# JinPLu/VeloxSeg

Hardware: AMD Instinct MI355X
Metric: training patches/s on 128^3 2-mod volumes (fwd+loss+bwd+allreduce+AdamW) (higher is better)
Workload: dtype f32

## Files before the change

include/veloxseg_hip.h:

```cpp
#ifndef VELOXSEG_HIP_H
#define VELOXSEG_HIP_H

#ifdef __cplusplus
extern "C" {
#endif

#define VX_ABI_VERSION 1

int vx_abi_version(void);
const char* vx_last_error(void);

int vx_conv3d_fwd(const float* x, const float* x2, int C1, const float* w, const float* bias, float* y,
                  int B, int Cin, int Di, int Hi, int Wi, int Cout, int K, int S, int P, int G, int ps, void* stream);
int vx_conv3d_bwd_data(const float* dy, const float* w, const float* bias_like, float* dx, float* dx2, int C1,
                       int B, int Cin, int Di, int Hi, int Wi, int Cout, int K, int S, int P, int G, int ps,
                       int accumulate, void* stream);
int vx_conv3d_bwd_weight(const float* x, const float* x2, int C1, const float* dy, float* dw, float* db,
                         int B, int Cin, int Di, int Hi, int Wi, int Cout, int K, int S, int P, int G, int ps, void* stream);

int vx_conv3d_bwd_weight_tiled(const float* x, const float* x2, int C1, const float* dy, float* dw, float* db,
                               int B, int Cin, int Di, int Hi, int Wi, int Cout, int K, int S, int P, int G, int ps, void* stream);
int vx_down_wgrad_ws_floats(int B, int Cin, int Di, int Hi, int Wi, int Cout);
int vx_down_wgrad_mfma(const float* x, const float* dy, float* dw, float* db, float* ws, long ws_floats,
                       int B, int Cin, int Di, int Hi, int Wi, int Cout, void* stream);
// ... 80 lines not shown
int vx_jlc_gk_h(const void* d_o, const void* y1, const void* y3, const void* y5, const float* stats_y, const float* part_t, void* g1, void* g3,
                void* g5, long BC, long V, int h16, void* stream);
int vx_mlp_fwd_h(const void* x, int norm, const double* part, int nparts, float* stats, const float* gamma, const float* beta,
                 const float* w1, const float* b1, const float* w2, const float* b2, float* out, int B, int C, int R, long V, float eps,
                 const void* seed_ptr, unsigned long long site1, float p1, unsigned long long site2, float p2, int h16, void* stream);
int vx_mlp_bwd_h(const void* x, int norm, const float* stats, const float* gamma, const float* beta, const float* w1, const float* b1,
                 const float* w2, const float* dout, void* dx, float* part_out, float* dgamma, float* dbeta, float* dw1, float* db1,
                 float* dw2, float* db2, int B, int C, int R, long V, float eps, const void* seed_ptr, unsigned long long site1, float p1,
                 unsigned long long site2, float p2, int h16, void* stream);

int vx_jlc_tz_ok(int C, int G, int D, int H, int W);
int vx_jlc_tz_ntiles(int C, int G, int D, int H, int W);
int vx_jlc_tz_img_floats(int C, int G);
int vx_jlc_tz_set_pieces(int ns);
int vx_jlc_tz_set_min_voxels(long v);
int vx_jlc_tz_pieces(void);
int vx_jlc_tz_set_debug(int mask);
int vx_jlc_tz_prep(const float* w1, const float* w3, const float* w5, float* img, int C, int G, void* stream);
int vx_jlc_tz_fwd(const float* x, const float* img, const float* b1, const float* b3, const float* b5, float* y1, float* y3, float* y5, double* part,
                  int B, int C, int G, int D, int H, int W, void* stream);
int vx_jlc_tz_bwd(const float* g1, const float* g3, const float* g5, const float* img, const float* w1, const float* d_o, float* dx,
                  int B, int C, int G, int D, int H, int W, void* stream);
int vx_jlc_cl_ok(int C, int G, int D, int H, int W);
int vx_jlc_cl_ntiles(int C, int G, int D, int H, int W);
int vx_jlc_cl_img_floats(int C, int G);
int vx_jlc_cl_set_enabled(int on);
int vx_jlc_cl_prep(const float* w1, const float* w3, const float* w5, float* img, int C, int G, void* stream);
int vx_jlc_cl_fwd(const float* x, const float* img, const float* b1, const float* b3, const float* b5, float* y1, float* y3, float* y5, double* part,
                  int B, int C, int G, int D, int H, int W, void* stream);
int vx_jlc_cl_bwd(const float* g1, const float* g3, const float* g5, const float* img, const float* d_o, float* dx, int B, int C, int G, int D, int H, int W,
                  void* stream);
int vx_jlc_wgrad_tz_ok(int C, int G, int D, int H, int W);
int vx_jlc_wgrad_tz_set_min_voxels(long v);
int vx_jlc_wgrad_tz_set_blocks(int n);
int vx_jlc_wgrad_tz_set_spec(int on);
int vx_jlc_wgrad_tz_set_f16(int on);
int vx_jlc_wgrad_tz(const float* x, const float* g1, const float* g3, const float* g5, float* dw1, float* dw3, float* dw5, int B, int C, int G, int D, int H, int W,
                    void* stream);
int vx_jlc_tz_img_floats_ns(int C, int G, int pieces);
int vx_jlc_tz_prep_ns(const float* w1, const float* w3, const float* w5, float* img, int C, int G, int pieces, void* stream);
int vx_jlc_tz_fwd_ns(const float* x, const float* img, const float* b1, const float* b3, const float* b5, float* y1, float* y3, float* y5, double* part,
                     int B, int C, int G, int D, int H, int W, int pieces, void* stream);
int vx_jlc_tz_bwd_ns(const float* g1, const float* g3, const float* g5, const float* img, const float* w1, const float* d_o, float* dx,
                     int B, int C, int G, int D, int H, int W, int pieces, void* stream);
int vx_jlc_wgrad_tz_ns(const float* x, const float* g1, const float* g3, const float* g5, float* dw1, float* dw3, float* dw5, int B, int C, int G, int D, int H, int W,
                       int pieces, void* stream);
int vx_jlc_tz_fwd_h(const float* x, const float* img, const float* b1, const float* b3, const float* b5, void* y1, void* y3, void* y5, double* part,
                    int B, int C, int G, int D, int H, int W, int pieces, int h16, void* stream);
int vx_jlc_tz_bwd_h(const void* g1, const void* g3, const void* g5, const float* img, const float* w1, const void* d_o, float* dx,
                    int B, int C, int G, int D, int H, int W, int pieces, int h16, void* stream);
int vx_jlc_wgrad_tz_h(const float* x, const void* g1, const void* g3, const void* g5, float* dw1, float* dw3, float* dw5, int B, int C, int G, int D, int H, int W,
                      int pieces, int h16, void* stream);

int vx_in_stats(const float* x, float* stats, double* part_ws, long BC, long V, float eps, void* stream);
int vx_in_apply_fwd(const float* y0, const float* y1, const float* y2, const float* s0, const float* s1, const float* s2,
                    int nk, int act, const float* res, float* out, long BC, long V, void* stream);
int vx_in_bwd(const float* dout, const float* y, const float* stats, int act, float* m_ws, double* part_ws, float* dy, long BC, long V, void* stream);
int vx_in_row_max(void);
int vx_in_row_fwd(const float* y0, const float* y1, const float* y2, float* s0, float* s1, float* s2, int nk, int act, const float* res,
                  float* out, long BC, long V, float eps, void* stream);
int vx_in_row_bwd(const float* dout, const float* y0, const float* y1, const float* y2, const float* s0, const float* s1, const float* s2,
                  int nk, int act, float* d0, float* d1, float* d2, long BC, long V, void* stream);
int vx_in_bwd_db(const float* dout, const float* y, const float* stats, int act, float* m_ws, double* part_ws, float* dy, long BC, long V, float* db, int C, void* stream);
int vx_in_fwd_split(const float* y0, const float* y1, const float* y2, float* s0, float* s1, float* s2, double* part_ws,
                    int nk, int act, const float* res, float* out, long BC, long V, float eps, void* stream);
int vx_in_bwd_split(const float* dout, const float* y0, const float* y1, const float* y2, const float* s0, const float* s1, const float* s2,
                    double* part_ws, int nk, int act, float* dy0, float* dy1, float* dy2, const float* add0, long BC, long V, void* stream);
int vx_in_row_bwd_add(const float* dout, const float* y0, const float* stats0, int act, const float* add0, float* d0, long BC, long V, void* stream);
int vx_in_row_bwd_db(const float* dout, const float* y0, const float* y1, const float* y2, const float* s0, const float* s1, const float* s2,
                     int nk, int act, float* d0, float* d1, float* d2, float* db0, float* db1, float* db2, int C, long BC, long V, void* stream);

int vx_ln_cf_fwd(const float* x, const float* gamma, const float* beta, float* out, int B, int C, long V, float eps, void* stream);
int vx_ln_cf_bwd(const float* x, const float* gamma, const float* dout, float* dx, float* dgamma, float* dbeta, float* ws,
                 int B, int C, long V, float eps, void* stream);
int vx_ln_cf_bwd_add(const float* x, const float* gamma, const float* dout, const float* add, float* dx, float* dgamma, float* dbeta, float* ws,
                     int B, int C, long V, float eps, void* stream);
int vx_ln_cf_bwd_data(const float* x, const float* gamma, const float* dout, const float* add, float* dx, float* ws, int B, int C, long V, float eps, void* stream);
int vx_ln_cf_bwd_param(const float* x, const float* dout, const float* ws, float* dgamma, float* dbeta, int B, int C, long V, void* stream);

int vx_gelu_drop_fwd(const float* a, float* h, long n, const void* seed_ptr, unsigned long long dstream, float p, void* stream);
int vx_gelu_drop_bwd(const float* dh, const float* a, float* da, long n, const void* seed_ptr, unsigned long long dstream, float p, void* stream);
int vx_axpy_drop_fwd(const float* x, const float* z, float* out, float alpha, long n, const void* seed_ptr, unsigned long long dstream, float p, void* stream);
int vx_axpy_drop_bwd(const float* dout, float* dx, float* dz, float alpha, long n, const void* seed_ptr, unsigned long long dstream, float p, void* stream);
int vx_add(const float* a, const float* b, const float* c, float* out, long n, void* stream);
int vx_add_many(const float* const* a, const float* const* b, const float* const* c, float* const* out, const long* n, int count, void* stream);
int vx_channel_sum(const float* dy, float* db, int B, int C, long V, void* stream);
int vx_space_to_depth2(const float* x, float* out, int B, int C, int Dc, int Hc, int Wc, int inverse, void* stream);
int vx_patchify(const float* x, float* out, int B, int C, int d, int h, int w, int K, void* stream);
int vx_patchify_bs(const float* x, long batch_stride, float* out, int B, int C, int d, int h, int w, int K, void* stream);
int vx_patchify_bs_h(const float* x, long batch_stride, void* out, int B, int C, int d, int h, int w, int K, int out_h16, void* stream);
int vx_patch_embed_ok(int Cin, int Cout, int Do, int Ho, int Wo, int K);
int vx_patch_embed_fwd(const float* x, long batch_stride, const float* w, const float* bias, float* y, int B, int Cin, int Cout, int Do, int Ho, int Wo, void* stream);
int vx_patch_embed_bwd_weight(const float* x, long batch_stride, const float* dy, float* dw, float* db, int B, int Cin, int Cout, int Do, int Ho, int Wo, void* stream);

typedef struct VxPwaPlan {
    int grid[3];
    int n[3];
    int heads, nb;
    int small[4][3];
    int nwin[4][3];
    int woff[4];
    int Ntot;
    int l;
} VxPwaPlan;

int vx_pwa_gather_fwd(const float* src, float* tok, const VxPwaPlan* plan, int c, int m, int M, int B, void* stream);
int vx_pwa_gather_bwd(const float* src, const float* dtok, float* dsrc, const VxPwaPlan* plan, int c, int m, int M, int B, void* stream);
int vx_pwa_gather_all_fwd(const float* const* srcs, float* tq, float* tk, float* tv, int* iq, int* ik, int* iv,
                          const VxPwaPlan* plan, int cq, int cv, int M, int B, void* stream);
int vx_pwa_gather_all_bwd(const float* dtq, const float* dtk, const float* dtv, const int* iq, const int* ik, const int* iv, float* const* dsrcs,
                          const VxPwaPlan* plan, int cq, int cv, int M, int B, void* stream);
int vx_pwa_scatter_fwd(const float* tok, float* out, const VxPwaPlan* plan, int c, int m, int M, int B, void* stream);
int vx_pwa_scatter_bwd(const float* dout, float* dtok, const VxPwaPlan* plan, int c, int m, int M, int B, void* stream);
int vx_pwa_scatter_fwd_all(const float* tok, float* const* outs, const VxPwaPlan* plan, int c, int M, int B, void* stream);
int vx_pwa_scatter_bwd_all(const float* const* douts, float* dtok, const VxPwaPlan* plan, int c, int M, int B, void* stream);
int vx_pwa_scatter_bwd_all_w(const float* const* douts, float* dtok, const VxPwaPlan* plan, int c, int M, int B, void* stream);
int vx_pwa_scatter_bwd_all_wz(const float* const* douts, float* dtok, const VxPwaPlan* plan, int c, int M, int B, float* extra_zero, long extra_floats, void* stream);
int vx_pwa_attn_set_fused_bwd(int on);
int vx_pwa_scatter_set_ident(int on);
int vx_pwa_attn_fwd(const float* Q, const float* K, const float* V, const float* table, float* O, float* LSE,
                    const VxPwaPlan* plan, int B, int M, int cq, int cv,
                    const void* seed_ptr, unsigned long long dstream, float p_drop, void* stream);
int vx_pwa_attn_bwd_ws_floats(const VxPwaPlan* plan, int B, int M);
int vx_pwa_attn_bwd_rep_offset(const VxPwaPlan* plan, int B, int M);
int vx_pwa_attn_bwd_mark_rep_zeroed(const float* delta_ws);
int vx_pwa_gather_set_vec(int on);
int vx_pwa_attn_bwd(const float* Q, const float* K, const float* V, const float* table, const float* O, const float* LSE,
                    const float* dO, float* dQ, float* dK, float* dV, float* dtable, float* delta_ws,
                    const VxPwaPlan* plan, int B, int M, int cq, int cv,
                    const void* seed_ptr, unsigned long long dstream, float p_drop, void* stream);
int vx_pwa_attn_bwd_nofold(const float* Q, const float* K, const float* V, const float* table, const float* O, const float* LSE,
                           const float* dO, float* dQ, float* dK, float* dV, float* delta_ws,
                           const VxPwaPlan* plan, int B, int M, int cq, int cv,
                           const void* seed_ptr, unsigned long long dstream, float p_drop, void* stream);
int vx_pwa_attn_bwd_fold(const float* delta_ws, float* dtable, const VxPwaPlan* plan, int B, int M, void* stream);
int vx_pwa_attn_bwd_fold_many(const float* const* delta_ws, float* const* dtables, const VxPwaPlan* const* plans, int count, int B, int M, void* stream);
int vx_pwa_attn_set_split(int S);
int vx_pwa_attn_bwd1_ok(const VxPwaPlan* plan, int B, int M, int cq, int cv);
int vx_pwa_attn_mbits_words(const VxPwaPlan* plan, int B, int M);
int vx_pwa_attn_mbits_useful(const VxPwaPlan* plan, int B, int M, int cq, int cv);
int vx_pwa_attn_set_valu_bits(int on);
int vx_pwa_attn_fwd_mb(const float* q, const float* k, const float* v, const float* table, float* out, float* lse, const VxPwaPlan* plan, int B, int M, int cq, int cv,
                       const void* seed_ptr, unsigned long long dstream, float p_drop, void* mbits, void* stream);
int vx_pwa_attn_bwd_mb(const float* q, const float* k, const float* v, const float* table, const float* out, const float* lse, const float* dout,
                       float* dq, float* dk, float* dv, float* dtable, float* delta_ws, const VxPwaPlan* plan, int B, int M, int cq, int cv,
                       const void* seed_ptr, unsigned long long dstream, float p_drop, const void* mbits, void* stream);
int vx_pwa_attn_bwd_nofold_mb(const float* q, const float* k, const float* v, const float* table, const float* out, const float* lse, const float* dout,
                              float* dq, float* dk, float* dv, float* delta_ws, const VxPwaPlan* plan, int B, int M, int cq, int cv,
                              const void* seed_ptr, unsigned long long dstream, float p_drop, const void* mbits, void* stream);
int vx_pwa_attn_mfma_ok(const VxPwaPlan* plan, int B, int M, int cq, int cv);
int vx_pwa_attn_set_mfma(int on);
int vx_pwa_attn_bwd1h_ok(const VxPwaPlan* plan, int B, int M, int cq, int cv);
int vx_pwa_attn_set_f16_bwd(int on);
int vx_pwa_attn_set_f16_bwd_ragged(int on);
int vx_pwa_attn_set_f16_bwd_m1(int on);
int vx_pwa_attn_set_short(int on);

int vx_seg_loss_fwd(const float* l0, const float* l1, const float* l2, const float* l3, int nh, const void* labels, int lab_kind,
                    double* acc, int B, int C, long V, void* stream);
int vx_sqdiff_sum(const float* a, const float* b, long n, double* acc, void* stream);
int vx_sqdiff_sum_bs(const float* a, const float* b, long n_per_sample, long b_batch_stride, int B, double* acc, void* stream);
int vx_mse_bwd_bs(const float* a, const float* b, long n_per_sample, long b_batch_stride, int B, const float* coef, const float* gout, float* da, void* stream);
int vx_sqdiff_sum_grad_bs(const float* a, const float* b, long n_per_sample, long b_batch_stride, int B, double* acc, float scale, float* da, void* stream);
int vx_sqdiff_sum_grad_bs_h(const void* a, const float* b, long n_per_sample, long b_batch_stride, int B, double* acc, float scale, void* da, int a_h16, void* stream);
int vx_loss_finalize(const double* seg_acc, int nh, int B, int C, long V, const float* head_weights,
                     const double* rc_acc, long n_rc, float w_rc,
                     const float* gram_seg, const float* g0, const float* g1, const float* g2, const float* g3, int M, int Cg, float w_f,
                     float* loss_out, float* coef, void* stream);
int vx_seg_loss_bwd(const float* logits, const void* labels, int lab_kind, const float* coef_head, const float* gout,
                    float* dlogits, int B, int C, long V, void* stream);
int vx_seg_loss_bwd4(const float* lg0, const float* lg1, const float* lg2, const float* lg3, int nh, const void* labels, int lab_kind, const float* coef,
                     int coef_stride, const float* gout, float* dl0, float* dl1, float* dl2, float* dl3, int B, int C, long V, void* stream);
int vx_seg_loss_ds_ok(int C, int D, int H, int W);
int vx_seg_loss_ds_set_columns(int on);
int vx_seg_loss_ds_ws_floats(const int* low_dims, int nh, int B, int C, int D);
int vx_seg_loss_ds_fwd(const float* l0, const float* l1, const float* l2, const float* l3, const int* low_dims, int nh, const void* labels, int lab_kind,
                       double* acc, int B, int C, int D, int H, int W, void* stream);
int vx_seg_loss_ds_bwd(const float* l0, const float* l1, const float* l2, const float* l3, const int* low_dims, int nh, const void* labels, int lab_kind,
                       const float* coef, int coef_stride, const float* gout, float* dl0, float* dl1, float* dl2, float* dl3, float* ws,
                       int B, int C, int D, int H, int W, void* stream);
int vx_seg_loss_ds_h16_ok(const int* low_dims, int nh, int B, int C, int D, int H, int W);
int vx_seg_loss_ds_fwd_h(const void* l0, const float* l1, const float* l2, const float* l3, const int* low_dims, int nh, const void* labels, int lab_kind,
                         double* acc, int B, int C, int D, int H, int W, int l0_h16, void* stream);
int vx_seg_loss_ds_bwd_h(const void* l0, const float* l1, const float* l2, const float* l3, const int* low_dims, int nh, const void* labels, int lab_kind,
                         const float* coef, int coef_stride, const float* gout, void* dl0, float* dl1, float* dl2, float* dl3, float* ws,
                         int B, int C, int D, int H, int W, int l0_h16, void* stream);
int vx_mse_bwd(const float* a, const float* b, const float* coef, const float* gout, float* da, long n, void* stream);
int vx_gram_mse_bwd(const float* gs, const float* g0, const float* g1, const float* g2, const float* g3, int M, const float* coef,
                    const float* gout, float* dgs, float* d0, float* d1, float* d2, float* d3, long n, void* stream);
int vx_gram_fwd(const float* x, float* G, int B, int C, long V, void* stream);
int vx_gram_bwd(const float* x, const float* dG, float* dx, int B, int C, long V, void* stream);
int vx_upsample_trilinear_fwd(const float* x, float* out, long BC, int d, int h, int w, int D, int H, int W, void* stream);
int vx_upsample_trilinear_bwd(const float* dout, float* dx, float* ws, long BC, int d, int h, int w, int D, int H, int W, void* stream);

int vx_upconv_set_mfma4(int on);
int vx_upconv_k2s2_fwd(const float* x, const float* w, const float* bias, float* y, int B, int Ci, int Co, int d, int h, int wd, void* stream);
int vx_upconv_k2s2_bwd_data(const float* dy, const float* w, float* dx, int B, int Ci, int Co, int d, int h, int wd, void* stream);
int vx_upconv_k2s2_wgrad_ok(int Ci, int Co);
int vx_upconv_k2s2_wgrad(const float* x, const float* dy, float* dw, int B, int Ci, int Co, int d, int h, int wd, void* stream);

int vx_adamw_step(float* p, const float* g, float* m, float* v, long n, float lr, float beta1, float beta2, float eps,
                  float weight_decay, long step, float grad_scale, void* stream);

int vx_sw_extract(const float* vol, float* win, int C, int D, int H, int W, int rd, int rh, int rw, int z0, int y0, int x0, void* stream);
int vx_sw_accumulate(const float* win, float* acc, int C, int D, int H, int W, int rd, int rh, int rw, int z0, int y0, int x0, float weight, void* stream);
int vx_sw_finalize(const float* acc, float* out, unsigned char* labels, const float* cz, const float* cy, const float* cx,
                   int C, int D, int H, int W, void* stream);
int vx_argmax_channels(const float* logits, unsigned char* labels, int B, int C, long V, void* stream);
int vx_confusion(const void* pred, int pred_bytes, const void* gt, int gt_bytes, unsigned long long* conf, int B, long V, int NC, void* stream);

int vx_min_value(const float* x, long n, float* out_init_inf, void* stream);
int vx_bbox_gt(const float* x, float thr, int C, int D, int H, int W, int* out6, void* stream);
int vx_label_chunk_count(const void* labels, int lab_bytes, long n, int chunk, int fg, int* counts, void* stream);
int vx_label_kth_in_chunk(const void* labels, int lab_bytes, long n, long chunk_start, int chunk, int fg, int k, long* out_index, void* stream);
int vx_rotate_z(const float* x, float* out, int C, int D, int H, int W, float cos_a, float sin_a, int mode, void* stream);

int vx_conv_mfma_ok(int Cin, int Cout, int D, int H, int W, int K, int S, int P, int G, int ps);
int vx_conv_mfma_set_stem_f16(int on);
int vx_conv_mfma_set_stem_pieces(int np);
int vx_conv_mfma_stem_pieces(void);
int vx_conv_mfma_ws_floats(int Cin, int Cout, int K, int backward);
int vx_conv_mfma_fwd(const float* x, const float* w, const float* bias, float* y, float* ws, int B, int Cin, int D, int H, int W, int Cout, int K, int S, int P,
                     void* stream);
int vx_conv_mfma_fwd_writes_absmax(int Cin, int Cout, int D, int H, int W, int K, int S, int P);
int vx_conv_mfma_fwd_mx(const float* x, const float* w, const float* bias, float* y, float* ws, unsigned* x_absmax, int B, int Cin, int D, int H, int W, int Cout,
                        int K, int S, int P, void* stream);
int vx_conv_mfma_bwd_data(const float* dy, const float* w, float* dx, float* ws, int B, int Cin, int D, int H, int W, int Cout, int K, int S, int P, int accumulate,
                          void* stream);

int vx_expand_split_ws_floats(int Cc, int ns);
int vx_expand_fwd_mfma_split(const float* x, const float* w, const float* bias, float* wt_ws, float* y, int B, int Cc, int D, int H, int W, int ns, void* stream);
int vx_expand_bwd_data_mfma_split(const float* dy_fine, const float* w, float* wt_ws, float* dx, int B, int Cc, int D, int H, int W, int accumulate, int ns, void* stream);
int vx_expand_split_ew_offset(int Cc);
int vx_expand_prep_split22(const float* w, float* wt_fwd, float* wt_bwd, int Cc, void* stream);
int vx_expand_fwd_mfma_split_prepared(const float* x, const float* bias, const float* wt_fwd, float* y, int B, int Cc, int D, int H, int W, void* stream);
int vx_expand_bwd_data_mfma_split_prepared(const float* dy_fine, const float* wt_bwd, const float* ew_fwd, float* dx, int B, int Cc, int D, int H, int W, int accumulate, void* stream);
int vx_expand_bwd_data_mfma_split_ew(const float* dy_fine, const float* w, float* wt_ws, float* dx, int B, int Cc, int D, int H, int W, int accumulate, int ns,
                                     const float* ew_fwd, void* stream);

int vx_ln_pw_ok(int C, int NS, const int* J, long V, int s2d);
int vx_ln_pw_tiles(int B, long V);
int vx_ln_pw_fwd(const void* const* ptrs, int M, int NS, const int* J, int B, int C, long V, float eps, int s2d, int gd, int gh, int gw, void* stream);
int vx_ln_pw_bwd(const void* const* ptrs, int M, int NS, const int* J, int B, int C, long V, float eps, int s2d, int gd, int gh, int gw, void* stream);
int vx_pwa_post_ok(int C, int Cv, int R, long V);
int vx_pwa_post_tiles(int B, long V);
int vx_pwa_post_fwd(const void* const* ptrs, int M, int B, int C, int Cv, int R, long V, float eps, float alpha, const void* seed_ptr, float p_mix, float p_ffn, void* stream);
int vx_pwa_post_bwd(const void* const* ptrs, int M, int B, int C, int Cv, int R, long V, float eps, float alpha, const void* seed_ptr, float p_mix, float p_ffn, void* stream);

int vx_inmlp_ok(int C, int R, long V);
int vx_inmlp_tiles(long V);
int vx_inmlp_fwd(const float* o, const double* part, int nparts, float* stats, const float* w1, const float* b1, const float* w2, const float* b2, float* out,
                 int B, int C, int R, long V, float eps, const void* seed_ptr, unsigned long long site, float p_drop, void* stream);
int vx_inmlp_bwd(const float* o, const float* stats, const float* w1, const float* b1, const float* w2, const float* dout, float* dn, float* part_dn,
                 float* sc_n, float* sc_h, float* sc_da, float* sc_dz, int B, int C, int R, long V, const void* seed_ptr, unsigned long long site, float p_drop,
                 void* stream);
int vx_pw_wgrad_group(const void* const* ptrs, const long* dims, int nj, const void* const* fptrs, const int* fdims, int nf, void* stream);

typedef struct VxTape VxTape;
int vx_tape_build(void* hip_graph, int max_lanes, VxTape** out);
int vx_tape_build_pgo(void* graph, int max_lanes, const float* dur_us, int n, VxTape** out);
int vx_tape_info(const VxTape* tape, int* n_nodes, int* n_kernels, int* n_lanes, int* n_events);
int vx_tape_set_lane_rotation(VxTape* tape, int k);
int vx_tape_replay(VxTape* tape, void* stream);
int vx_tape_free(VxTape* tape);
int vx_tape_flag_set(void* flag, int value, void* stream);
int vx_tape_flag_wait(const void* flag, int value, void* stream);
int vx_tape_set_flags(int on);
int vx_tape_set_flag_timeout_ms(int ms);
int vx_tape_flag_timeouts(void);
int vx_tape_hop(int slot, void* src, void* dst);
int vx_tape_mark(int id, void* stream);
int vx_tape_wait_marker(VxTape* tape, int id, void* stream);
int vx_tape_has_marker(const VxTape* tape, int id);
int vx_tape_profile(VxTape* tape, void* stream, int reps, float* us);
int vx_tape_describe(const VxTape* tape, int* lane, int* grid, int* waits4, char* names, int name_stride);
int vx_tape_waits(const VxTape* tape, int* waits, int stride);
int vx_tape_launch_node(VxTape* tape, int node, void* stream);
int vx_tape_set_fuzz(int seed, float max_us, float prob);
int vx_tape_node_param(const VxTape* tape, int node, int k, int nparams, int size, void* out, int cap, int* got);
int vx_tape_node_kind(const VxTape* tape, int node);
int vx_tape_replay_prefix(VxTape* tape, void* stream, int k);
int vx_tape_lane_stream(void* any_stream, int lane, void** out);
int vx_spin_us(float us, void* stream);
int vx_tape_lanes_distinct(void);
int vx_tape_spin_us(void);
int vx_tape_lane_on_caller_queue(void);
int vx_tape_permute_lanes(const int* perm4);

#ifdef __cplusplus
}
#endif
#endif
```

veloxseg_amd/csrc/pwa_mfma.hip:

```cpp
#include "vx_common.h"
#include <stdlib.h>
#include "../../include/veloxseg_hip.h"

typedef float vx_f32x4 __attribute__((ext_vector_type(4)));
#define VX_MFMA(a, b, c) __builtin_amdgcn_mfma_f32_16x16x4f32((a), (b), (c), 0, 0, 0)
#define VX_DTABLE_REPLICAS 16

struct VxAttnM {
    int BH, heads, Nt, ML, l, M;
    int n[3];
    float scale;
    int lin_cst, Tsz;
    int xcd;
};

__device__ __forceinline__ void vx_am_tables(const VxAttnM& A, const float* __restrict__ table, int a, int* lin, float* bias, int nthr) {
    for (int t = threadIdx.x; t < A.l; t += nthr) {
        const int t2 = t % A.n[2], t1 = (t / A.n[2]) % A.n[1], t0 = t / (A.n[2] * A.n[1]);
        lin[t] = (t0 * (2 * A.n[1] - 1) + t1) * (2 * A.n[2] - 1) + t2;
    }
    for (int k0 = threadIdx.x; k0 < A.Tsz; k0 += nthr * 8) {
        float v[8];
#pragma unroll
        for (int u = 0; u < 8; ++u) { const int k = k0 + u * nthr; v[u] = table[(long)(k < A.Tsz ? k : 0) * A.heads + a]; }
// ... 930 lines not shown
#pragma unroll
            for (int g = 0; g < MF; ++g)
#pragma unroll
                for (int f = 0; f < MF; ++f) mkc[g][f] = mk[g][f];
            if (j + 1 < NTq) load_bits(j + 1);
            float dssum[4] = {0.f, 0.f, 0.f, 0.f};
            bool pv[4];
#pragma unroll
            for (int i = 0; i < 4; ++i) pv[i] = !RAG || (kval && 16 * qt + 4 * qg + i < A.l);
            uint32_t pmh[2][4], pml[2][4], dsh[2][4], dsl[2][4];
            if constexpr (MF == 1) {
#pragma unroll
                for (int e = 2; e < 4; ++e) { pmh[0][e] = 0u; pml[0][e] = 0u; dsh[0][e] = 0u; dsl[0][e] = 0u; }
            }
#pragma unroll
            for (int g = 0; g < MF; ++g) {
                const _Float16* rrow = rq + (g * nq + 16 * j + m) * VX_BH_RS;
                const vx_au4 aS = *reinterpret_cast<const vx_au4*>(rrow + poffS), aP = *reinterpret_cast<const vx_au4*>(rrow + poffP);
                const float4 l4 = *reinterpret_cast<const float4*>(&lse_s[g * nq + 16 * j + 4 * qg]);
                const float4 d4 = *reinterpret_cast<const float4*>(&del_s[g * nq + 16 * j + 4 * qg]);
                const float bl[4] = {bs[0] - l4.x, bs[1] - l4.y, bs[2] - l4.z, bs[3] - l4.w}, del[4] = {d4.x, d4.y, d4.z, d4.w};
                vx_f32x4 sv_[2], dp[2];
#pragma unroll
                for (int f = 0; f < MF; ++f) {
                    sv_[f] = VX_MFMA_H(aS, kop[f], ((vx_f32x4){0.f, 0.f, 0.f, 0.f}));
                    dp[f] = VX_MFMA_H(aP, vop[f], ((vx_f32x4){0.f, 0.f, 0.f, 0.f}));
                }
#pragma unroll
                for (int f = 0; f < MF; ++f) {
                    float pm[4], ds[4];
#pragma unroll
                    for (int i = 0; i < 4; ++i) {
                        float p = __builtin_amdgcn_exp2f(fmaf(sv_[f][i], cS, bl[i]));
                        if (RAG) p = pv[i] ? p : 0.0f;
                        float mkf = 1.0f;
                        if constexpr (DROP) {
                            const uint32_t w = (i < 2) ? mkc[g][f].x : mkc[g][f].y;
                            mkf = ((w >> (m + 16 * (i & 1))) & 1u) ? keepf : 0.0f;
                        }
                        pm[i] = p * mkf;
                        ds[i] = p * fmaf(dp[f][i], mkf, -del[i]);
                        dssum[i] += ds[i];
                    }
                    vx_a_split2(pm[0], pm[1], pmh[f][2 * g], pml[f][2 * g]);
                    vx_a_split2(pm[2], pm[3], pmh[f][2 * g + 1], pml[f][2 * g + 1]);
                    vx_a_split2(ds[0], ds[1], dsh[f][2 * g], dsl[f][2 * g]);
                    vx_a_split2(ds[2], ds[3], dsh[f][2 * g + 1], dsl[f][2 * g + 1]);
                }
                __builtin_amdgcn_wave_barrier();
#pragma unroll
                for (int f = 0; f < MF; ++f)
#pragma unroll
                    for (int i = 0; i < 4; ++i) {
                        const uint32_t h = dsh[f][2 * g + (i >> 1)], l = dsl[f][2 * g + (i >> 1)];
                        tr[f * (16 * TS) + (4 * qg + i) * TS + m] = (i & 1) ? __builtin_amdgcn_perm(l, h, 0x07060302u) : __builtin_amdgcn_perm(l, h, 0x05040100u);
                    }
                __builtin_amdgcn_wave_barrier();
                const vx_au4 r0 = *reinterpret_cast<const vx_au4*>(&tr[m * TS + 4 * qg]);
                const vx_au4 r1 = MF == 2 ? *reinterpret_cast<const vx_au4*>(&tr[16 * TS + m * TS + 4 * qg]) : (vx_au4){0u, 0u, 0u, 0u};
                __builtin_amdgcn_wave_barrier();
                const vx_au4 bh = {__builtin_amdgcn_perm(r0[1], r0[0], 0x05040100u), __builtin_amdgcn_perm(r0[3], r0[2], 0x05040100u),
                                   __builtin_amdgcn_perm(r1[1], r1[0], 0x05040100u), __builtin_amdgcn_perm(r1[3], r1[2], 0x05040100u)};
                const vx_au4 bl_ = {__builtin_amdgcn_perm(r0[1], r0[0], 0x07060302u), __builtin_amdgcn_perm(r0[3], r0[2], 0x07060302u),
                                    __builtin_amdgcn_perm(r1[1], r1[0], 0x07060302u), __builtin_amdgcn_perm(r1[3], r1[2], 0x07060302u)};
                vx_f32x4 dqT = VX_MFMA_H(kth, bh, ((vx_f32x4){0.f, 0.f, 0.f, 0.f}));
                dqT = VX_MFMA_H(ktl, bh, dqT);
                dqT = VX_MFMA_H(kth, bl_, dqT);
                if (4 * qg < C) {
                    float4* dst = reinterpret_cast<float4*>(&dqm[(g * nq + 16 * j + m) * C + 4 * qg]);
                    float4 o4 = *dst;
                    o4.x += dqT[0]; o4.y += dqT[1]; o4.z += dqT[2]; o4.w += dqT[3];
                    *dst = o4;
                }
            }
            {
                const _Float16* tcol = tq + m * VX_BH_TS + 16 * j + 4 * qg;
                const uint2 q0 = *reinterpret_cast<const uint2*>(tcol), q1 = *reinterpret_cast<const uint2*>(tcol + nq);
                const uint2 o0 = *reinterpret_cast<const uint2*>(tcol + 16 * VX_BH_TS), o1 = *reinterpret_cast<const uint2*>(tcol + 16 * VX_BH_TS + nq);
                const vx_au4 aQ = {q0.x, q0.y, q1.x, q1.y}, aO = {o0.x, o0.y, o1.x, o1.y};
#pragma unroll
                for (int f = 0; f < MF; ++f) {
                    dv[f] = VX_MFMA_H(aO, ((vx_au4){pmh[f][0], pmh[f][1], pmh[f][2], pmh[f][3]}), dv[f]);
                    dv[f] = VX_MFMA_H(aO, ((vx_au4){pml[f][0], pml[f][1], pml[f][2], pml[f][3]}), dv[f]);
                    dk[f] = VX_MFMA_H(aQ, ((vx_au4){dsh[f][0], dsh[f][1], dsh[f][2], dsh[f][3]}), dk[f]);
                    dk[f] = VX_MFMA_H(aQ, ((vx_au4){dsl[f][0], dsl[f][1], dsl[f][2], dsl[f][3]}), dk[f]);
                }
            }
#pragma unroll
            for (int i = 0; i < 4; ++i) { if (kval) gw[raw[i] - wbase] += dssum[i]; __builtin_amdgcn_wave_barrier(); }
        }
        const float fK = A.scale * ldexpf(1.0f, -(eq + ed + ev)), fV = ldexpf(1.0f, -ed), fQ = A.scale * ldexpf(1.0f, -(ek + ed + ev)), fB = ldexpf(1.0f, -(ed + ev));
#pragma unroll
        for (int f = 0; f < MF; ++f)
#pragma unroll
            for (int i = 0; i < 4; ++i) { totk[f][i] = fmaf(dk[f][i], fK, totk[f][i]); totv[f][i] = fmaf(dv[f][i], fV, totv[f][i]); }
        __syncthreads();
        constexpr int img = NR * C;
        for (int e = threadIdx.x; e < img; e += 256) {
            const int c = e % C, r2 = e / C, f = r2 / nq, t = 16 * q_lo + (r2 - f * nq);
            float* dst = dQ + (wrow + (long)f * A.l + t) * C + c;
            const float v = ((dqw[e] + dqw[img + e]) + (dqw[2 * img + e] + dqw[3 * img + e])) * fQ;
            dqw[e] = 0.0f; dqw[img + e] = 0.0f; dqw[2 * img + e] = 0.0f; dqw[3 * img + e] = 0.0f;
            if ((RAG && t >= A.l) || f >= MF) continue;
            if (atomic_dq) atomicAdd(dst, v); else *dst = v;
        }
        {
            const int* wb_s = reinterpret_cast<const int*>(red) + 16;
            constexpr int NU = RAG ? 4 : 2;
            float gsum[NU];
#pragma unroll
            for (int u = 0; u < NU; ++u) {
                const int x = threadIdx.x + 256 * u;
                float g = 0.0f;
                if (x < 2 * WIN) {
#pragma unroll
                    for (int w = 0; w < 4; ++w) {
                        const int y = x - wb_s[w];
                        if (y >= 0 && y < WIN) g += (gwin[(4 * w) * WIN + y] + gwin[(4 * w + 1) * WIN + y]) + (gwin[(4 * w + 2) * WIN + y] + gwin[(4 * w + 3) * WIN + y]);
                    }
                }
                gsum[u] = g;
            }
            __syncthreads();
#pragma unroll
            for (int u = 0; u < NU; ++u) {
                const int x = threadIdx.x + 256 * u;
                const int k = bbase + x + A.lin_cst;
                if (gsum[u] != 0.0f && k >= 0 && k < A.Tsz) atomicAdd(dtab_dst + (long)k * A.heads + a, gsum[u] * fB);
            }
            for (int e = threadIdx.x; e < 16 * WIN; e += 256) gwin[e] = 0.0f;
        }
    }
#pragma unroll
    for (int f = 0; f < MF; ++f) {
        const long kr = wrow + (long)f * A.l + kcc;
        float k4[4], v4[4];
#pragma unroll
        for (int i = 0; i < 4; ++i) {
            k4[i] = totk[f][i] + __shfl_xor(totk[f][i], 4 * C, 64);
            v4[i] = totv[f][i] + __shfl_xor(totv[f][i], 4 * C, 64);
        }
        if (4 * qg < C && kval) {
            if (QS == 1) {
                *reinterpret_cast<float4*>(dK + kr * C + 4 * qg) = make_float4(k4[0], k4[1], k4[2], k4[3]);
                *reinterpret_cast<float4*>(dV + kr * C + 4 * qg) = make_float4(v4[0], v4[1], v4[2], v4[3]);
            } else {
#pragma unroll
                for (int i = 0; i < 4; ++i) { atomicAdd(dK + kr * C + 4 * qg + i, k4[i]); atomicAdd(dV + kr * C + 4 * qg + i, v4[i]); }
            }
        }
    }
}

static bool vx_am_fill(VxAttnM& A, const VxPwaPlan* P, int B, int M, int cq) {
    A.BH = B * P->heads; A.heads = P->heads; A.Nt = P->Ntot; A.l = P->l; A.M = M; A.ML = M * P->l;
    A.n[0] = P->n[0]; A.n[1] = P->n[1]; A.n[2] = P->n[2];
    A.scale = 1.0f / sqrtf((float)cq);
    A.lin_cst = ((P->n[0] - 1) * (2 * P->n[1] - 1) + (P->n[1] - 1)) * (2 * P->n[2] - 1) + (P->n[2] - 1);
    A.Tsz = (2 * A.n[0] - 1) * (2 * A.n[1] - 1) * (2 * A.n[2] - 1);
    static const int xcd = [] { const char* e = getenv("VELOXSEG_ATTN_XCD"); return e ? atoi(e) : 3; }();
    A.xcd = xcd;
    return true;
}
static size_t vx_am_tab_floats(const VxAttnM& A) { return (size_t)((A.l + 3) & ~3) + (size_t)((A.Tsz + 3) & ~3); }
static size_t vx_am_lds_fwd(const VxAttnM& A, int cq, int cv) { return (vx_am_tab_floats(A) + (size_t)A.ML * cq + (size_t)A.ML * (cv + 2)) * 4; }
static size_t vx_am_lds_q(const VxAttnM& A, int cq, int cv) { return (vx_am_tab_floats(A) + (size_t)4 * ((A.Tsz + 3) & ~3) + (size_t)A.ML * (cq + cv)) * 4; }
static size_t vx_am_lds_kv(const VxAttnM& A, int cq, int cv) { return (vx_am_tab_floats(A) + (size_t)A.ML * (cq + cv + 2)) * 4; }

static int vx_am_enabled = 3;
extern "C" int vx_pwa_attn_set_mfma(int mask) { vx_am_enabled = mask & 15; return 0; }

extern "C" int vx_pwa_attn_mfma_ok(const VxPwaPlan* P, int B, int M, int cq, int cv) {
    const int want = (vx_am_enabled & 1) | ((vx_am_enabled & 4) ? 2 : 0);
    if (!want || P == nullptr || B <= 0 || M <= 0) return 0;
    if (P->l % 64 != 0 || cq % 4 != 0 || cq > 16 || cv % 4 != 0 || cv > 32) return 0;
    if (!((cq == 4 && cv == 4) || (cq == 8 && cv == 8) || (cq == 8 && cv == 16) || (cq == 16 && cv == 32) || (cq == 16 && cv == 16) || (cq == 4 && cv == 8))) return 0;
    VxAttnM A;
    vx_am_fill(A, P, B, M, cq);
    const size_t cap = 150 * 1024;
    return (vx_am_lds_fwd(A, cq, cv) <= cap && vx_am_lds_q(A, cq, cv) <= cap && vx_am_lds_kv(A, cq, cv) <= cap) ? want : 0;
}

template <int A_, int B_> struct vx_am_pair { static constexpr int a = A_, b = B_; };
template <class F> static bool vx_am_dispatch(int cq, int cv, F&& f) {
#define VX_CASE(X, Y) if (cq == X && cv == Y) { f(vx_am_pair<X, Y>{}); return true; }
    VX_CASE(4, 4) VX_CASE(8, 8) VX_CASE(8, 16) VX_CASE(16, 32) VX_CASE(16, 16) VX_CASE(4, 8)
#undef VX_CASE
    return false;
}
template <class K> static void vx_am_attr(K kernel) { (void)hipFuncSetAttribute((const void*)kernel, hipFuncAttributeMaxDynamicSharedMemorySize, 160 * 1024); }

int vx_pwa_attn_mfma_fwd(const float* Q, const float* K, const float* V, const float* table, float* O, float* LSE, unsigned short* mbits, const VxPwaPlan* plan, int B, int M,
                         int cq, int cv, VxDrop d, void* stream) {
    VxAttnM A;
    vx_am_fill(A, plan, B, M, cq);
    const dim3 grid(vx_cdiv(A.ML / 16, 8), (unsigned)((long)A.BH * A.Nt));
    const size_t shm = vx_am_lds_fwd(A, cq, cv);
    vx_am_dispatch(cq, cv, [&](auto pr) {
        constexpr int CQ = decltype(pr)::a, CV = decltype(pr)::b;
        static bool once = false;
        if (!once) { vx_am_attr(vx_pwa_attn_mfma_fwd_k<CQ, CV>); once = true; }
        vx_pwa_attn_mfma_fwd_k<CQ, CV><<<grid, dim3(512), shm, (hipStream_t)stream>>>(Q, K, V, table, O, LSE, A, d, mbits);
    });
    return 0;
}
int vx_pwa_attn_mfma_bwd(const float* Q, const float* K, const float* V, const float* table, const float* O, const float* LSE, const float* dO, float* dQ,
                         float* dK, float* dV, float* dtable, float* delta, float* rep, const VxPwaPlan* plan, int B, int M, int cq, int cv, VxDrop d,
                         void* stream) {
    VxAttnM A;
    vx_am_fill(A, plan, B, M, cq);
    const dim3 grid(vx_cdiv(A.ML / 16, 8), (unsigned)((long)A.BH * A.Nt));
    const size_t shm_q = vx_am_lds_q(A, cq, cv), shm_kv = vx_am_lds_kv(A, cq, cv);
    vx_am_dispatch(cq, cv, [&](auto pr) {
        constexpr int CQ = decltype(pr)::a, CV = decltype(pr)::b;
        static bool once = false;
        if (!once) { vx_am_attr(vx_pwa_attn_mfma_bwd_q_k<CQ, CV>); vx_am_attr(vx_pwa_attn_mfma_bwd_kv_k<CQ, CV>); once = true; }
        vx_pwa_attn_mfma_bwd_q_k<CQ, CV><<<grid, dim3(512), shm_q, (hipStream_t)stream>>>(Q, K, V, table, O, LSE, dO, dQ, delta, rep, A, d);
        vx_pwa_attn_mfma_bwd_kv_k<CQ, CV><<<grid, dim3(512), shm_kv, (hipStream_t)stream>>>(Q, K, V, table, LSE, delta, dO, dK, dV, rep, dtable, A, d);
    });
    return 0;
}

struct VxB1Geo { int NT, waves_used, nbx, QS, NTq, win; size_t shm; };
static int vx_b1_span(const VxAttnM& A, int ntok, int step) {
    int worst = 0;
    for (int t0 = 0; t0 < A.l; t0 += step) {
        int lo = 1 << 30, hi = -(1 << 30);
        for (int t = t0; t < t0 + ntok; ++t) {
            const int tc = t < A.l ? t : A.l - 1;
            const int t2 = tc % A.n[2], t1 = (tc / A.n[2]) % A.n[1], tz = tc / (A.n[2] * A.n[1]);
            const int v = (tz * (2 * A.n[1] - 1) + t1) * (2 * A.n[2] - 1) + t2;
            lo = v < lo ? v : lo; hi = v > hi ? v : hi;
        }
        worst = (hi - lo) > worst ? (hi - lo) : worst;
    }
    return worst;
}
static VxB1Geo vx_b1_geo(const VxAttnM& A, int cq, int mf, bool few_windows = false) {
    VxB1Geo g;
    g.NT = (A.l + 15) / 16;
    g.waves_used = g.NT < 4 ? g.NT : 4;
    g.nbx = (g.NT + g.waves_used - 1) / g.waves_used;
    g.NTq = g.NT < 4 ? g.NT : 4;
    if (few_windows) g.NTq = 1;
    while (g.NT % g.NTq) --g.NTq;
    g.QS = g.NT / g.NTq;
    const int sq = vx_b1_span(A, g.NTq * 16, g.NTq * 16), sk16 = vx_b1_span(A, 16, 16), sk64 = vx_b1_span(A, 16 * g.waves_used, 16 * g.waves_used);
    g.win = (sq + sk16 + 1 <= VX_B1_WIN && sq + sk64 + 1 <= 2 * VX_B1_WIN) ? 1 : 0;
    const size_t lp = (size_t)g.NT * 16, nq = (size_t)g.NTq * 16, tpad = (size_t)((A.Tsz + 3) & ~3);
    g.shm = (lp + (g.win ? 2 * VX_B1_WIN + 4 * VX_B1_WIN : 2 * tpad) + 2 * mf * nq + 4 * mf * nq * cq + (size_t)4 * mf * 16 * 20) * sizeof(float);
    return g;
}
struct VxZeroMany { float4* p[4]; long n4[4]; };
__global__ void __launch_bounds__(256) vx_zero_many_k(VxZeroMany z) {
    float4* __restrict__ p = z.p[blockIdx.y];
    const long n = z.n4[blockIdx.y];
#pragma unroll
    for (int u = 0; u < 4; ++u) {
        const long i = ((long)blockIdx.x * 4 + u) * 256 + threadIdx.x;
        if (i < n) p[i] = make_float4(0.f, 0.f, 0.f, 0.f);
    }
}
static bool vx_b1_short(const VxAttnM& A) { return A.M == 1 && A.l < 512; }
static int g_b1_short = -1;
static int vx_b1_short_on() { if (g_b1_short < 0) g_b1_short = getenv("VELOXSEG_B1_SHORT") ? atoi(getenv("VELOXSEG_B1_SHORT")) : 1; return g_b1_short; }
extern "C" int vx_pwa_attn_set_short(int on) { g_b1_short = on ? 1 : 0; return 0; }
static bool vx_b1_few(const VxAttnM& A) {
    static const int on = getenv("VELOXSEG_B1_FEW") ? atoi(getenv("VELOXSEG_B1_FEW")) : -1;
    const int NT = (A.l + 15) / 16;
    const bool use = on >= 0 ? on != 0 : (vx_b1_short_on() && vx_b1_short(A) && A.l % 16 == 0);
    return use && NT >= 2 && (long)A.BH * A.Nt * ((NT + 3) / 4) * ((NT + 3) / 4) < 64;
}
extern "C" int vx_pwa_attn_bwd1_ok(const VxPwaPlan* P, int B, int M, int cq, int cv) {
    if (!(vx_am_enabled & 10) || (vx_am_enabled & 4) || P == nullptr || B <= 0 || M < 1 || M > 2) return 0;
    if (!((cq == 4 && cv == 4) || (cq == 8 && cv == 8) || (cq == 8 && cv == 16) || (cq == 16 && cv == 32) || (cq == 16 && cv == 16) || (cq == 4 && cv == 8))) return 0;
    VxAttnM A;
    vx_am_fill(A, P, B, M, cq);
    const bool prefer = (vx_am_enabled & 8) || P->l % 16 != 0 || vx_b1_few(A) || (vx_b1_short_on() && vx_b1_short(A));
    if (!prefer) return 0;
    return vx_b1_geo(A, cq, M, vx_b1_few(A)).shm <= 80 * 1024 ? 1 : 0;
}
int vx_pwa_attn_bwd1(const float* Q, const float* K, const float* V, const float* table, const float* O, const float* LSE, const float* dO, float* dQ,
                     float* dK, float* dV, float* rep, const unsigned short* mbits, const VxPwaPlan* plan, int B, int M, int cq, int cv, VxDrop d, void* stream) {
    VxAttnM A;
    vx_am_fill(A, plan, B, M, cq);
    const long nwin = (long)A.BH * A.Nt;
    const VxB1Geo g = vx_b1_geo(A, cq, M, vx_b1_few(A));
    const dim3 grid((unsigned)(g.nbx * g.QS), (unsigned)nwin);
    const int atomic_dq = g.nbx > 1 ? 1 : 0;
    hipStream_t st = (hipStream_t)stream;
    const long rows = nwin * A.ML;
    if (atomic_dq || g.QS > 1) {
        VxZeroMany z = {};
        int nz = 0;
        if (atomic_dq) { z.p[nz] = reinterpret_cast<float4*>(dQ); z.n4[nz] = rows * cq / 4; ++nz; }
        if (g.QS > 1) { z.p[nz] = reinterpret_cast<float4*>(dK); z.n4[nz] = rows * cq / 4; ++nz; z.p[nz] = reinterpret_cast<float4*>(dV); z.n4[nz] = rows * cv / 4; ++nz; }
        long mx = 0;
        for (int i = 0; i < nz; ++i) mx = z.n4[i] > mx ? z.n4[i] : mx;
        vx_zero_many_k<<<dim3((unsigned)vx_cdiv(mx, 256 * 4), (unsigned)nz), dim3(256), 0, st>>>(z);
    }
    vx_am_dispatch(cq, cv, [&](auto pr) {
        constexpr int CQ = decltype(pr)::a, CV = decltype(pr)::b;
        const bool al = (A.l & 3) == 0;
#define VX_B1(MF_, AL_, WIN_)                                                                                                         \
        {                                                                                                                             \
            static bool once = false;                                                                                                 \
            if (!once) {                                \
                if (hipFuncSetAttribute((const void*)vx_pwa_attn_bwd1_k<CQ, CV, MF_, AL_, WIN_>, hipFuncAttributeMaxDynamicSharedMemorySize, 96 * 1024) != hipSuccess) (void)hipGetLastError(); \
                once = true;                                                                                                          \
            }                                                                                                                         \
            vx_pwa_attn_bwd1_k<CQ, CV, MF_, AL_, WIN_><<<grid, dim3(256), g.shm, st>>>(Q, K, V, table, O, LSE, dO, dQ, dK, dV, rep, A, d, g.waves_used, atomic_dq, \
                                                                                      g.QS, g.NTq, mbits);                         \
        }
#define VX_B1W(MF_, AL_) { if (g.win) VX_B1(MF_, AL_, true) else VX_B1(MF_, AL_, false) }
        if (M == 1) { if (al) VX_B1W(1, true) else VX_B1W(1, false) }
        else { if (al) VX_B1W(2, true) else VX_B1W(2, false) }
#undef VX_B1W
#undef VX_B1
    });
    return 0;
}

static int vx_am_f16_bwd = 1;
extern "C" int vx_pwa_attn_set_f16_bwd(int on) { vx_am_f16_bwd = on ? 1 : 0; return 0; }
static size_t vx_b1h_shm(int LP, int Tsz, int win, int c) {
    return ((size_t)LP + (size_t)((Tsz + 3) & ~3) + 16 * (size_t)win + 2 * 128 + (size_t)4 * 128 * c + 4 * 2 * 16 * 20 + 32) * sizeof(float) + ((size_t)128 * VX_BH_RS + 2 * 16 * VX_BH_TS) * 2;
}
static size_t vx_b1h_shm(const VxAttnM& A, int c) { return vx_b1h_shm(A.l, A.Tsz, VX_B1_WIN, c); }
struct VxB1hRag { int LP, win; };
static int g_b1h_rag = -1;
extern "C" int vx_pwa_attn_set_f16_bwd_ragged(int on) { g_b1h_rag = on < 0 ? 0 : on; return 0; }
static VxB1hRag vx_b1h_rag(const VxAttnM& A, int c) {
    VxB1hRag r = {0, 0};
    if (g_b1h_rag < 0) g_b1h_rag = getenv("VELOXSEG_F16_BWD_RAGGED") ? atoi(getenv("VELOXSEG_F16_BWD_RAGGED")) : 1;
    if (!g_b1h_rag || A.l < 8) return r;
    const int LP = (A.l + 63) / 64 * 64;
    if (g_b1h_rag == 1 && A.l * 4 < LP * 3) return r;
    const int sq = vx_b1_span(A, 64, 64), sk16 = vx_b1_span(A, 16, 16), sk64 = vx_b1_span(A, 64, 64);
    int win = (sq + sk16 + 1 + 63) / 64 * 64;
    if (win < VX_B1_WIN) win = VX_B1_WIN;
    while (sq + sk64 + 1 > 2 * win) win += 64;
    if (win > 512 || vx_b1h_shm(LP, A.Tsz, win, c) > 80 * 1024) return r;
    r.LP = LP; r.win = win;
    return r;
}
static int g_b1h_m1 = -1;
extern "C" int vx_pwa_attn_set_f16_bwd_m1(int on) { g_b1h_m1 = on < 0 ? 0 : on; return 0; }
extern "C" int vx_pwa_attn_bwd1h_ok(const VxPwaPlan* P, int B, int M, int cq, int cv) {
    if (!vx_am_f16_bwd || !(vx_am_enabled & 2) || (vx_am_enabled & 4) || P == nullptr || B <= 0 || M < 1 || M > 2) return 0;
// ... 61 lines not shown
```

Measured before the change: 1068.

## Add split-f16 MFMA forward kernel for small-head windowed attention

Adds a new forward attention kernel for head widths 4 and 8. K, V, Q and the probabilities are each split into high and low f16 parts with per-block power-of-two scaling, so the QK and PV products run on f16 MFMA while keeping close to f32 accuracy. K and V are stored in LDS as compact f16 images, with V kept transposed. The kernel is enabled by default, except for M==1 which needs an environment variable. It replaces the f32 16x16x4 MFMA forward path, at the cost of extra split arithmetic and possible precision differences.

```diff
diff --git a/include/veloxseg_hip.h b/include/veloxseg_hip.h
--- a/include/veloxseg_hip.h
+++ b/include/veloxseg_hip.h
@@ -256,6 +256,8 @@
 int vx_pwa_attn_set_mfma(int on);
 int vx_pwa_attn_bwd1h_ok(const VxPwaPlan* plan, int B, int M, int cq, int cv);
 int vx_pwa_attn_set_f16_bwd(int on);
+int vx_pwa_attn_set_f16_fwd(int on);
+int vx_pwa_attn_fwd1h_ok(const VxPwaPlan* plan, int B, int M, int cq, int cv);
 int vx_pwa_attn_set_f16_bwd_ragged(int on);
 int vx_pwa_attn_set_f16_bwd_m1(int on);
 int vx_pwa_attn_set_short(int on);
diff --git a/veloxseg_amd/csrc/pwa_mfma.hip b/veloxseg_amd/csrc/pwa_mfma.hip
--- a/veloxseg_amd/csrc/pwa_mfma.hip
+++ b/veloxseg_amd/csrc/pwa_mfma.hip
@@ -1106,6 +1106,180 @@
     }
 }
 
+template <int CQ, int CV>
+__global__ void __launch_bounds__(512, 4) vx_pwa_attn_fwd1h_k(const float* __restrict__ Q, const float* __restrict__ K, const float* __restrict__ Vt,
+                                                              const float* __restrict__ table, float* __restrict__ O, float* __restrict__ LSE,
+                                                              VxAttnM A, VxDrop drop, unsigned short* __restrict__ mbits) {
+    static_assert(CQ == CV && (CQ == 4 || CQ == 8), "head widths (4, 4) and (8, 8)");
+    constexpr int C = CQ, NPT = 4;
+    constexpr float LOG2E = 1.4426950408889634f;
+    extern __shared__ __attribute__((aligned(16))) float vx_am_lds[];
+    int* __restrict__ lin = reinterpret_cast<int*>(vx_am_lds);
+    float* __restrict__ bias = vx_am_lds + ((A.l + 3) & ~3);
+    float* __restrict__ red = bias + ((A.Tsz + 3) & ~3);
+    _Float16* __restrict__ kimg = reinterpret_cast<_Float16*>(red + 16);
+    _Float16* __restrict__ vimg = kimg + A.ML * 2 * C;
+    const int VS = A.ML + 8;
+    int bx_, by_;
+    vx_xcd_rows(bx_, by_, A.xcd & 1);
+    const long win = by_;
+    const int a = (int)((win / A.Nt) % A.heads);
+    const float* __restrict__ kp = K + win * A.ML * C;
+    const float* __restrict__ vp = Vt + win * A.ML * C;
+    const int n4 = A.ML * (C / 4);
+    float4 k4[NPT], v4[NPT];
+#pragma unroll
+    for (int u = 0; u < NPT; ++u) {
+        const int e = threadIdx.x + u * 512;
+        k4[u] = reinterpret_cast<const float4*>(kp)[e < n4 ? e : 0];
+        v4[u] = reinterpret_cast<const float4*>(vp)[e < n4 ? e : 0];
+    }
+    const int lane = threadIdx.x & 63, wave = threadIdx.x >> 6, m = lane & 15, qg = lane >> 4;
+    const int q0 = (bx_ * 8 + wave) * 16;
+    const bool qv = q0 < A.ML;
+    const long row = win * A.ML + (qv ? q0 + m : 0);
+    float qx[C];
+#pragma unroll
+    for (int c4 = 0; c4 < C / 4; ++c4) {
+        const float4 t = *reinterpret_cast<const float4*>(Q + row * C + 4 * c4);
+        qx[4 * c4] = t.x; qx[4 * c4 + 1] = t.y; qx[4 * c4 + 2] = t.z; qx[4 * c4 + 3] = t.w;
+    }
+    vx_am_tables(A, table, a, lin, bias, 512);
+    for (int k = threadIdx.x; k < A.Tsz; k += 512) bias[k] *= LOG2E;
+    float kmx = 0.0f, vmx = 0.0f;
+#pragma unroll
+    for (int u = 0; u < NPT; ++u) {
+        if (threadIdx.x + u * 512 < n4) {
+            kmx = fmaxf(kmx, fmaxf(fmaxf(fabsf(k4[u].x), fabsf(k4[u].y)), fmaxf(fabsf(k4[u].z), fabsf(k4[u].w))));
+            vmx = fmaxf(vmx, fmaxf(fmaxf(fabsf(v4[u].x), fabsf(v4[u].y)), fmaxf(fabsf(v4[u].z), fabsf(v4[u].w))));
+        }
+    }
+    kmx = vx_wave_max(kmx); vmx = vx_wave_max(vmx);
+    if (lane == 0) { red[wave] = kmx; red[8 + wave] = vmx; }
+    __syncthreads();
+    kmx = red[0]; vmx = red[8];
+#pragma unroll
+    for (int w = 1; w < 8; ++w) { kmx = fmaxf(kmx, red[w]); vmx = fmaxf(vmx, red[8 + w]); }
+    const int ek = vx_a_exp(kmx, 10), ev = vx_a_exp(vmx, 10);
+    {
+        const float sk = ldexpf(1.0f, ek), sv = ldexpf(1.0f, ev);
+#pragma unroll
+        for (int u = 0; u < NPT; ++u) {
+            const int e = threadIdx.x + u * 512;
+            if (e < n4) {
+                const int key = e / (C / 4), c4 = e - key * (C / 4);
+                const int it = key >> 6, w = key & 63, tu = (w >> 2) & 3, mrow = 4 * (w >> 4) + (w & 3);
+                uint32_t h0, h1, l0, l1;
+                vx_a_split2(k4[u].x * sk, k4[u].y * sk, h0, l0);
+                vx_a_split2(k4[u].z * sk, k4[u].w * sk, h1, l1);
+                uint32_t* d = reinterpret_cast<uint32_t*>(kimg + ((4 * it + tu) * 16 + mrow) * 2 * C + 4 * c4);
+                *reinterpret_cast<uint2*>(d) = make_uint2(h0, h1);
+                *reinterpret_cast<uint2*>(d + C / 2) = make_uint2(l0, l1);
+                vx_a_split2(v4[u].x * sv, v4[u].y * sv, h0, l0);
+                vx_a_split2(v4[u].z * sv, v4[u].w * sv, h1, l1);
+                unsigned short* vt = reinterpret_cast<unsigned short*>(vimg) + (4 * c4) * VS + key;
+                vt[0] = (unsigned short)(h0 & 0xffffu); vt[VS] = (unsigned short)(h0 >> 16); vt[2 * VS] = (unsigned short)(h1 & 0xffffu); vt[3 * VS] = (unsigned short)(h1 >> 16);
+                vt += C * VS;
+                vt[0] = (unsigned short)(l0 & 0xffffu); vt[VS] = (unsigned short)(l0 >> 16); vt[2 * VS] = (unsigned short)(l1 & 0xffffu); vt[3 * VS] = (unsigned short)(l1 >> 16);
+            }
+        }
+    }
+    __syncthreads();
+    if (!qv) return;
+    const VxDropCtx dc = vx_attn_ctx(drop);
+    vx_au4 qop;
+    float cS;
+    {
+        float qmx = 0.0f;
+#pragma unroll
+        for (int c = 0; c < C; ++c) qmx = fmaxf(qmx, fabsf(qx[c]));
+        const int eq = vx_a_exp(qmx, 10);
+        const float sq = ldexpf(1.0f, eq);
+        cS = A.scale * LOG2E * ldexpf(1.0f, -(eq + ek));
+        uint32_t h[C / 2], l[C / 2];
+#pragma unroll
+        for (int c = 0; c < C; c += 2) vx_a_split2(qx[c] * sq, qx[c + 1] * sq, h[c / 2], l[c / 2]);
+        if constexpr (C == 8) {
+            const bool lo_ = (qg & 1) != 0;
+            qop = (vx_au4){lo_ ? l[0] : h[0], lo_ ? l[1] : h[1], lo_ ? l[2] : h[2], lo_ ? l[3] : h[3]};
+        } else {
+            qop = qg == 0 ? (vx_au4){h[0], h[1], h[0], h[1]} : (qg == 1 ? (vx_au4){l[0], l[1], l[0], l[1]} : (vx_au4){0u, 0u, 0u, 0u});
+        }
+    }
+    const int lin_q = lin[(q0 + m) % A.l] + A.lin_cst;
+    const int koff = C == 8 ? 8 * (qg >> 1) : 0;
+    const bool vrow = m < 2 * C;
+    float mrun = -INFINITY, lsum = 0.0f;
+    vx_f32x4 oacc = {0.f, 0.f, 0.f, 0.f}, oacc2 = {0.f, 0.f, 0.f, 0.f};
+    const int nit = A.ML >> 6;
+#pragma unroll 1
+    for (int it = 0; it < nit; ++it) {
+        const int kt0 = 4 * it;
+        vx_f32x4 s[4];
+        int4 lk[4];
+#pragma unroll
+        for (int u = 0; u < 4; ++u) {
+            lk[u] = *reinterpret_cast<const int4*>(&lin[(16 * (kt0 + qg)) % A.l + 4 * u]);
+            const vx_au4 ka = *reinterpret_cast<const vx_au4*>(kimg + ((kt0 + u) * 16 + m) * 2 * C + koff);
+            s[u] = VX_MFMA_H(ka, qop, ((vx_f32x4){0.f, 0.f, 0.f, 0.f}));
+        }
+        vx_au4 va[2];
+#pragma unroll
+        for (int h = 0; h < 2; ++h) va[h] = vrow ? *reinterpret_cast<const vx_au4*>(vimg + m * VS + 64 * it + 16 * qg + 8 * h) : (vx_au4){0u, 0u, 0u, 0u};
+        float mt = -INFINITY;
+#pragma unroll
+        for (int u = 0; u < 4; ++u) {
+            s[u][0] = fmaf(s[u][0], cS, bias[lin_q - lk[u].x]); s[u][1] = fmaf(s[u][1], cS, bias[lin_q - lk[u].y]);
+            s[u][2] = fmaf(s[u][2], cS, bias[lin_q - lk[u].z]); s[u][3] = fmaf(s[u][3], cS, bias[lin_q - lk[u].w]);
+            mt = fmaxf(mt, fmaxf(fmaxf(s[u][0], s[u][1]), fmaxf(s[u][2], s[u][3])));
+        }
+        mt = fmaxf(mt, __shfl_xor(mt, 16, 64));
+        mt = fmaxf(mt, __shfl_xor(mt, 32, 64));
+        const float mn = fmaxf(mrun, mt);
+        const float alpha = __builtin_amdgcn_exp2f(mrun - mn);
+        mrun = mn;
+        float m16[16];
+        vx_attn_drop16(dc, (uint64_t)row * (uint64_t)A.ML + (uint64_t)(16 * (kt0 + qg)), m16);
+        if (mbits != nullptr && dc.on) {
+            unsigned w = 0;
+#pragma unroll
+            for (int e = 0; e < 16; ++e) w |= (m16[e] != 0.0f ? 1u : 0u) << e;
+            mbits[(win * (A.ML >> 4) + (kt0 + qg)) * A.ML + q0 + m] = (unsigned short)w;
+        }
+        float psum = 0.0f;
+#pragma unroll
+        for (int u = 0; u < 4; ++u) {
+#pragma unroll
+            for (int i = 0; i < 4; ++i) { const float p = __builtin_amdgcn_exp2f(s[u][i] - mn); psum += p; s[u][i] = m16[4 * u + i] != 0.0f ? p : 0.0f; }
+        }
+        lsum = lsum * alpha + psum;
+        oacc *= alpha; oacc2 *= alpha;
+        uint32_t ph[2][4], pl[2][4];
+#pragma unroll
+        for (int h = 0; h < 2; ++h) {
+            vx_a_split2(s[2 * h][0], s[2 * h][1], ph[h][0], pl[h][0]);
+            vx_a_split2(s[2 * h][2], s[2 * h][3], ph[h][1], pl[h][1]);
+            vx_a_split2(s[2 * h + 1][0], s[2 * h + 1][1], ph[h][2], pl[h][2]);
+            vx_a_split2(s[2 * h + 1][2], s[2 * h + 1][3], ph[h][3], pl[h][3]);
+        }
+        oacc = VX_MFMA_H(va[0], ((vx_au4){ph[0][0], ph[0][1], ph[0][2], ph[0][3]}), oacc);
+        oacc2 = VX_MFMA_H(va[1], ((vx_au4){ph[1][0], ph[1][1], ph[1][2], ph[1][3]}), oacc2);
+        oacc = VX_MFMA_H(va[0], ((vx_au4){pl[0][0], pl[0][1], pl[0][2], pl[0][3]}), oacc);
+        oacc2 = VX_MFMA_H(va[1], ((vx_au4){pl[1][0], pl[1][1], pl[1][2], pl[1][3]}), oacc2);
+    }
+    oacc += oacc2;
+    lsum += __shfl_xor(lsum, 16, 64);
+    lsum += __shfl_xor(lsum, 32, 64);
+    float o[4];
+#pragma unroll
+    for (int i = 0; i < 4; ++i) o[i] = oacc[i] + __shfl_xor(oacc[i], 4 * C, 64);
+    if (4 * qg < C) {
+        const float f = dc.inv_keep * ldexpf(1.0f, -ev) / lsum;
+        *reinterpret_cast<float4*>(O + row * C + 4 * qg) = make_float4(o[0] * f, o[1] * f, o[2] * f, o[3] * f);
+    }
+    if (qg == 0) LSE[row] = (mrun + log2f(lsum)) * 0.6931471805599453f;
+}
+
 static bool vx_am_fill(VxAttnM& A, const VxPwaPlan* P, int B, int M, int cq) {
     A.BH = B * P->heads; A.heads = P->heads; A.Nt = P->Ntot; A.l = P->l; A.M = M; A.ML = M * P->l;
     A.n[0] = P->n[0]; A.n[1] = P->n[1]; A.n[2] = P->n[2];
@@ -1144,11 +1318,39 @@
 }
 template <class K> static void vx_am_attr(K kernel) { (void)hipFuncSetAttribute((const void*)kernel, hipFuncAttributeMaxDynamicSharedMemorySize, 160 * 1024); }
 
+static int vx_am_f16_fwd = -1;
+extern "C" int vx_pwa_attn_set_f16_fwd(int on) { vx_am_f16_fwd = on < 0 ? 0 : (on > 2 ? 2 : on); return 0; }
+static size_t vx_f1h_shm(const VxAttnM& A, int c) {
+    return ((size_t)((A.l + 3) & ~3) + (size_t)((A.Tsz + 3) & ~3) + 16) * sizeof(float) + ((size_t)A.ML * 2 * c + (size_t)2 * c * (A.ML + 8)) * 2;
+}
+static bool vx_f1h_ok(const VxAttnM& A, int cq, int cv) {
+    if (vx_am_f16_fwd < 0) vx_am_f16_fwd = (getenv("VELOXSEG_F16_FWD_M1") && atoi(getenv("VELOXSEG_F16_FWD_M1"))) ? 2 : 1;
+    if (!vx_am_f16_fwd || cq != cv || (cq != 4 && cq != 8) || A.l % 64 != 0 || (A.M == 1 && vx_am_f16_fwd < 2)) return false;
+    return A.ML * cq <= 8192 && vx_f1h_shm(A, cq) <= 150 * 1024;
+}
+extern "C" int vx_pwa_attn_fwd1h_ok(const VxPwaPlan* P, int B, int M, int cq, int cv) {
+    if (!(vx_pwa_attn_mfma_ok(P, B, M, cq, cv) & 1)) return 0;
+    VxAttnM A;
+    vx_am_fill(A, P, B, M, cq);
+    return vx_f1h_ok(A, cq, cv) ? 1 : 0;
+}
+
 int vx_pwa_attn_mfma_fwd(const float* Q, const float* K, const float* V, const float* table, float* O, float* LSE, unsigned short* mbits, const VxPwaPlan* plan, int B, int M,
                          int cq, int cv, VxDrop d, void* stream) {
     VxAttnM A;
     vx_am_fill(A, plan, B, M, cq);
     const dim3 grid(vx_cdiv(A.ML / 16, 8), (unsigned)((long)A.BH * A.Nt));
+    if (vx_f1h_ok(A, cq, cv)) {
+        const size_t shm = vx_f1h_shm(A, cq);
+        auto go = [&](auto kernel, bool& once) {
+            if (!once) { vx_am_attr(kernel); once = true; }
+            kernel<<<grid, dim3(512), shm, (hipStream_t)stream>>>(Q, K, V, table, O, LSE, A, d, mbits);
+        };
+        static bool once4 = false, once8 = false;
+        if (cq == 8) go(vx_pwa_attn_fwd1h_k<8, 8>, once8);
+        else go(vx_pwa_attn_fwd1h_k<4, 4>, once4);
+        return 0;
+    }
     const size_t shm = vx_am_lds_fwd(A, cq, cv);
     vx_am_dispatch(cq, cv, [&](auto pr) {
         constexpr int CQ = decltype(pr)::a, CV = decltype(pr)::b;
```

Result: no change. 1070 (median of 6 runs) (+0.1%).
